# SavaRobotics/FoundationPose

Measured on AMD Instinct MI355X. Metric: pose-hypotheses/sec (render+refine+score), 252 hyp x 160x160, higher is better.
Workload: dtype f16

## Files before the change

foundationpose_amd/csrc/head_mlp.hip:

```cpp
#include "common.h"
#include "device_util.h"
#include <cstdlib>

#define HM_THREADS 512
#define HM_TILE 65536
#define HM_RED_OFF (2 * HM_TILE)
#define HM_LDS_BYTES (2 * HM_TILE + 4096)

struct HmCtx {
  int lane, wave, lr, lh;
  unsigned xo[8];
};

__device__ __forceinline__ void hm_gemm(const HmCtx &c, const f16 *w, const float *bias, const unsigned char *tile, floatx16 (&acc)[2][2]) {
  acc_from_bias(acc, bias, c.wave * 64, c.lh);
  const u32x4 *wp = reinterpret_cast<const u32x4 *>(w) + (size_t)(c.wave >> 1) * (32 * 4 * 64) + ((c.wave & 1) * 2) * 64 + c.lane;
  constexpr int D = 4;
  u32x4 wr[D][2];
#pragma unroll
  for (int d = 0; d < D; ++d)
#pragma unroll
    for (int i = 0; i < 2; ++i) wr[d][i] = wp[(d * 4 + i) * 64];
  const unsigned char *xb = tile + c.lr * 256;
  half8 bf[2][2];
#pragma unroll
  for (int j = 0; j < 2; ++j) bf[0][j] = *reinterpret_cast<const half8 *>(xb + j * 8192 + c.xo[0]);
#pragma unroll
  for (int k = 0; k < 32; ++k) {
    const int cur = k & 1, slot = k % D;
    half8 af[2];
#pragma unroll
    for (int i = 0; i < 2; ++i) af[i] = *reinterpret_cast<half8 *>(&wr[slot][i]);
    __builtin_amdgcn_sched_barrier(0);
    if (k + D < 32) {
#pragma unroll
      for (int i = 0; i < 2; ++i) wr[slot][i] = wp[((k + D) * 4 + i) * 64];
    }
    if (k + 1 < 32) {
      const int kn = k + 1;
#pragma unroll
      for (int j = 0; j < 2; ++j) bf[cur ^ 1][j] = *reinterpret_cast<const half8 *>(xb + (kn >> 3) * 16384 + j * 8192 + c.xo[kn & 7]);
    }
    __builtin_amdgcn_sched_barrier(0);
#pragma unroll
    for (int j = 0; j < 2; ++j)
#pragma unroll
      for (int i = 0; i < 2; ++i) acc[i][j] = __builtin_amdgcn_mfma_f32_32x32x16_f16(af[i], bf[cur][j], acc[i][j], 0, 0, 0);
  }
}

__device__ __forceinline__ unsigned hm_off(const HmCtx &c, int row, int i, int rg) {
  return (unsigned)((c.wave >> 1) * 16384 + row * 256 + ((((c.wave & 1) * 8 + i * 4 + rg) ^ (row & 15)) * 16) + c.lh * 8);
}

__device__ __forceinline__ void hm_residual_stats(const HmCtx &c, const unsigned char *res_tile, float *red, floatx16 (&acc)[2][2], float (&rstd)[2]) {
#pragma unroll
  for (int j = 0; j < 2; ++j) {
    const int row = j * 32 + c.lr;
#pragma unroll
    for (int i = 0; i < 2; ++i)
#pragma unroll
      for (int rg = 0; rg < 4; ++rg) {
        const half4 rq = *reinterpret_cast<const half4 *>(res_tile + hm_off(c, row, i, rg));
#pragma unroll
        for (int e = 0; e < 4; ++e) acc[i][j][rg * 4 + e] += (float)rq[e];
      }
  }
  float mean[2];
#pragma unroll
  for (int j = 0; j < 2; ++j) {
    float s = 0.f;
#pragma unroll
    for (int i = 0; i < 2; ++i)
#pragma unroll
      for (int e = 0; e < 16; ++e) s += acc[i][j][e];
    s += __shfl_xor(s, 32);
    if (c.lh == 0) red[c.wave * 64 + j * 32 + c.lr] = s;
  }
  __syncthreads();
#pragma unroll
  for (int j = 0; j < 2; ++j) {
    float s = 0.f;
#pragma unroll
    for (int w = 0; w < 8; ++w) s += red[w * 64 + j * 32 + c.lr];
    mean[j] = s * (1.f / 512.f);
  }
#pragma unroll
  for (int j = 0; j < 2; ++j) {
    float s = 0.f;
#pragma unroll
    for (int i = 0; i < 2; ++i)
#pragma unroll
      for (int e = 0; e < 16; ++e) {
        acc[i][j][e] -= mean[j];
        s += acc[i][j][e] * acc[i][j][e];
      }
    s += __shfl_xor(s, 32);
    if (c.lh == 0) red[512 + c.wave * 64 + j * 32 + c.lr] = s;
  }
  __syncthreads();
#pragma unroll
  for (int j = 0; j < 2; ++j) {
    float s = 0.f;
#pragma unroll
    for (int w = 0; w < 8; ++w) s += red[512 + w * 64 + j * 32 + c.lr];
    rstd[j] = rsqrtf(s * (1.f / 512.f) + 1e-5f);
  }
}

__global__ __launch_bounds__(HM_THREADS, 1) void head_mlp_kernel(HeadMlpArgs p) {
  extern __shared__ __attribute__((aligned(16))) unsigned char hm_smem[];
  HmCtx c;
  const int tid = threadIdx.x;
  c.lane = tid & 63;
  c.wave = __builtin_amdgcn_readfirstlane(tid >> 6);
  c.lr = c.lane & 31;
  c.lh = c.lane >> 5;
#pragma unroll
  for (int s = 0; s < 8; ++s) c.xo[s] = (unsigned)(((2 * s + c.lh) ^ (c.lr & 15)) * 16);
  const int m0 = blockIdx.x * 64;
  unsigned char *P = hm_smem, *Q = hm_smem + HM_TILE;
  float *red = reinterpret_cast<float *>(hm_smem + HM_RED_OFF);
  const unsigned lds0 = (unsigned)(size_t)(__attribute__((address_space(3))) void *)hm_smem;

  tok_tile_dma<64, 8>(p.att, m0, p.M, c.wave, c.lane, lds0);
  tok_tile_dma<64, 8>(p.tok, m0, p.M, c.wave, c.lane, lds0 + HM_TILE);
  wait_vm<8>();
  __syncthreads();

  floatx16 acc[2][2];
  float rstd[2];
  hm_gemm(c, p.w_out, p.b_out, P, acc);
  wait_vm<0>();
  __syncthreads();
  hm_residual_stats(c, Q, red, acc, rstd);
#pragma unroll
  for (int i = 0; i < 2; ++i)
#pragma unroll
    for (int rg = 0; rg < 4; ++rg) {
      const int col = c.wave * 64 + i * 32 + rg * 8 + c.lh * 4;
      const float4 gv = *reinterpret_cast<const float4 *>(p.g1 + col), bv = *reinterpret_cast<const float4 *>(p.be1 + col);
#pragma unroll
      for (int j = 0; j < 2; ++j) {
        half4 hv;
        hv[0] = (f16)(acc[i][j][rg * 4 + 0] * rstd[j] * gv.x + bv.x);
        hv[1] = (f16)(acc[i][j][rg * 4 + 1] * rstd[j] * gv.y + bv.y);
        hv[2] = (f16)(acc[i][j][rg * 4 + 2] * rstd[j] * gv.z + bv.z);
        hv[3] = (f16)(acc[i][j][rg * 4 + 3] * rstd[j] * gv.w + bv.w);
        *reinterpret_cast<half4 *>(Q + hm_off(c, j * 32 + c.lr, i, rg)) = hv;
      }
    }
  __syncthreads();
  hm_gemm(c, p.w1, p.b1, Q, acc);
#pragma unroll
  for (int i = 0; i < 2; ++i)
#pragma unroll
    for (int rg = 0; rg < 4; ++rg)
#pragma unroll
      for (int j = 0; j < 2; ++j) {
        half4 hv;
#pragma unroll
        for (int e = 0; e < 4; ++e) hv[e] = (f16)acc[i][j][rg * 4 + e];
        hv = __builtin_elementwise_max(hv, half4{(f16)0.f, (f16)0.f, (f16)0.f, (f16)0.f});
        *reinterpret_cast<half4 *>(P + hm_off(c, j * 32 + c.lr, i, rg)) = hv;
      }
  __syncthreads();
  hm_gemm(c, p.w2, p.b2, P, acc);
  hm_residual_stats(c, Q, red, acc, rstd);
#pragma unroll
  for (int j = 0; j < 2; ++j)
#pragma unroll
    for (int i = 0; i < 2; ++i)
#pragma unroll
      for (int rg = 0; rg < 4; ++rg) {
        float v[4];
#pragma unroll
        for (int e = 0; e < 4; ++e) v[e] = row16_sum(acc[i][j][rg * 4 + e] * rstd[j]);
        const int g = (m0 + j * 32 + (c.lr & 16)) >> 4;
        if ((c.lr & 15) == 0 && g * 16 < p.M)
          *reinterpret_cast<float4 *>(p.gsum + (size_t)g * 512 + c.wave * 64 + i * 32 + rg * 8 + c.lh * 4) = make_float4(v[0], v[1], v[2], v[3]);
      }
}


#define H2_ROWS 128
#ifdef HM_STAMP
__device__ unsigned long long g_hm_stamps[1024 * 8 * 8];
extern "C" __attribute__((visibility("default"))) int fp_dbg_hm_stamps(unsigned long long *host) {
  return hipMemcpyFromSymbol(host, HIP_SYMBOL(g_hm_stamps), sizeof(g_hm_stamps)) == hipSuccess ? 0 : -1;
}
#define HSTAMP(i) do { if (blockIdx.x < 1024 && c.lane == 0) g_hm_stamps[((size_t)blockIdx.x * 8 + c.wave) * 8 + (i)] = __builtin_amdgcn_s_memtime(); } while (0)
#else
#define HSTAMP(i) do { } while (0)
#endif
#define H2_SEG (H2_ROWS * 256)
#define H2_TILE (4 * H2_SEG)
#define H2_SLOT (H2_ROWS * 128)
#define H2_RING_OFF H2_TILE
#define H2_RED_OFF H2_RING_OFF
#define H2_LDS_BYTES (H2_TILE + 2 * H2_SLOT)

__device__ __forceinline__ void h2_ring_dma(const f16 *src, int m0, int M, int s8, int wave, int lane, unsigned slot_addr) {
#pragma unroll
  for (int u = 0; u < 2; ++u) {
    const int r8 = wave * 2 + u, row = r8 * 8 + (lane >> 3);
    const int m = min(m0 + row, M - 1);
    const unsigned voff = (unsigned)(((size_t)m * 512 + s8 * 64 + (((lane & 7) ^ (row & 7)) * 8)) * 2);
    glds16(src, voff, slot_addr + r8 * 1024);
  }
}

struct H2Ctx {
  int lane, wave, lr, lh;
};

template <bool RING, bool BIAS, typename Pre>
__device__ __forceinline__ void h2_gemm(const H2Ctx &c, const f16 *w, const float *bias, const unsigned char *smem, floatx16 (&acc)[2][4], Pre before_loop,
                                        unsigned lds0 = 0, const f16 *ring_src = nullptr, int m0 = 0, int M = 0) {
  const u32x4 *wp = reinterpret_cast<const u32x4 *>(w) + (size_t)(c.wave >> 1) * (32 * 4 * 64) + ((c.wave & 1) * 2) * 64 + c.lane;
  constexpr int D = 3;
  u32x4 wr[D][2];
#pragma unroll
  for (int d = 0; d < D; ++d)
#pragma unroll
    for (int i = 0; i < 2; ++i) wr[d][i] = wp[(d * 4 + i) * 64];
  __builtin_amdgcn_sched_barrier(0);
  if constexpr (RING) {
    wait_vm<6>();
    __syncthreads();
    h2_ring_dma(ring_src, m0, M, 1, c.wave, c.lane, lds0 + H2_RING_OFF + H2_SLOT);
  }
  floatx16 bvec[2];
  if constexpr (BIAS) {
#pragma unroll
    for (int i = 0; i < 2; ++i)
#pragma unroll
      for (int rg = 0; rg < 4; ++rg) {
        const float4 bv = *reinterpret_cast<const float4 *>(bias + c.wave * 64 + i * 32 + rg * 8 + c.lh * 4);
        bvec[i][rg * 4 + 0] = bv.x, bvec[i][rg * 4 + 1] = bv.y, bvec[i][rg * 4 + 2] = bv.z, bvec[i][rg * 4 + 3] = bv.w;
      }
  }
  __builtin_amdgcn_sched_barrier(0);
  before_loop();
  const unsigned char *xb = RING ? smem + H2_RING_OFF + c.lr * 128 + ((c.lh ^ (c.lr & 1)) * 16) : smem + c.lr * 256 + ((c.lh ^ (c.lr & 1)) * 16);
  const unsigned xe = (unsigned)(c.lr & (RING ? 6 : 14));
  auto frag_addr = [&](int k, int j) __attribute__((always_inline)) -> const unsigned char * {
    if constexpr (RING) return xb + ((k >> 2) & 1) * H2_SLOT + j * 4096 + (((unsigned)(2 * (k & 3)) ^ xe) << 4);
    else return xb + (k >> 3) * H2_SEG + j * 8192 + (((unsigned)(2 * (k & 7)) ^ xe) << 4);
  };
  half8 bf[4];
#pragma unroll
  for (int j = 0; j < 4; ++j) bf[j] = *reinterpret_cast<const half8 *>(frag_addr(0, j));
#pragma unroll
  for (int k = 0; k < 32; ++k) {
    const int slot = k % D;
    half8 af[2];
#pragma unroll
    for (int i = 0; i < 2; ++i) af[i] = *reinterpret_cast<half8 *>(&wr[slot][i]);
    __builtin_amdgcn_sched_barrier(0);
    if (k + D < 32) {
#pragma unroll
      for (int i = 0; i < 2; ++i) wr[slot][i] = wp[((k + D) * 4 + i) * 64];
    }
    __builtin_amdgcn_sched_barrier(0);
    const int kn = k + 1;
    const bool seg_edge = RING && (kn & 3) == 0 && kn < 32;
#pragma unroll
    for (int j = 0; j < 4; ++j) {
#pragma unroll
      for (int i = 0; i < 2; ++i) acc[i][j] = __builtin_amdgcn_mfma_f32_32x32x16_f16(af[i], bf[j], (BIAS && k == 0) ? bvec[i] : acc[i][j], 0, 0, 0);
      __builtin_amdgcn_sched_barrier(0);
      if (kn < 32 && !seg_edge) bf[j] = *reinterpret_cast<const half8 *>(frag_addr(kn, j));
      __builtin_amdgcn_sched_barrier(0);
    }
    if (seg_edge) {
      wait_vm_lgkm<8>();
      __syncthreads();
      if ((kn >> 2) + 1 < 8) h2_ring_dma(ring_src, m0, M, (kn >> 2) + 1, c.wave, c.lane, lds0 + H2_RING_OFF + (((kn >> 2) + 1) & 1) * H2_SLOT);
#pragma unroll
      for (int j = 0; j < 4; ++j) bf[j] = *reinterpret_cast<const half8 *>(frag_addr(kn, j));
    }
  }
}

__device__ __forceinline__ unsigned h2_off(const H2Ctx &c, int row, int i, int rg) {
  return (unsigned)((c.wave >> 1) * H2_SEG + row * 256 + ((((c.wave & 1) * 8 + i * 4 + rg) ^ (row & 15)) * 16) + c.lh * 8);
}
__device__ __forceinline__ H2Ctx h2_fresh(const H2Ctx &c0) {
  H2Ctx c = c0;
  asm volatile("" : "+v"(c.lr), "+v"(c.lh), "+v"(c.lane));
  return c;
}

__device__ __forceinline__ void h2_stats(const H2Ctx &c0, float *red, const floatx16 (&acc)[2][4], float (&mean)[4], float (&rstd)[4]) {
  H2Ctx c = c0;
  asm volatile("" : "+v"(c.lr));
#pragma unroll
  for (int j = 0; j < 4; ++j) {
    float s = 0.f, q = 0.f;
#pragma unroll
    for (int i = 0; i < 2; ++i)
#pragma unroll
      for (int e = 0; e < 16; ++e) {
        s += acc[i][j][e];
        q += acc[i][j][e] * acc[i][j][e];
      }
    s += __shfl_xor(s, 32);
    q += __shfl_xor(q, 32);
    if (c.lh == 0) *reinterpret_cast<float2 *>(&red[(c.wave * 128 + j * 32 + c.lr) * 2]) = make_float2(s, q);
  }
  __syncthreads();
#pragma unroll
  for (int j = 0; j < 4; ++j) {
    float s = 0.f, q = 0.f;
#pragma unroll
    for (int w = 0; w < 8; ++w) {
      const float2 v = *reinterpret_cast<const float2 *>(&red[(w * 128 + j * 32 + c.lr) * 2]);
      s += v.x;
      q += v.y;
    }
    mean[j] = s * (1.f / 512.f);
    rstd[j] = rsqrtf(fmaxf(q * (1.f / 512.f) - mean[j] * mean[j], 0.f) + 1e-5f);
  }
}

__global__ __launch_bounds__(HM_THREADS, 1) void head_mlp128_kernel(HeadMlpArgs p) {
  extern __shared__ __attribute__((aligned(16))) unsigned char h2_smem[];
  H2Ctx c;
  const int tid = threadIdx.x;
  c.lane = tid & 63;
  c.wave = __builtin_amdgcn_readfirstlane(tid >> 6);
  c.lr = c.lane & 31;
  c.lh = c.lane >> 5;
  const int m0 = blockIdx.x * H2_ROWS;
  unsigned char *Q = h2_smem;
  float *red = reinterpret_cast<float *>(h2_smem + H2_RED_OFF);
  const unsigned lds0 = (unsigned)(size_t)(__attribute__((address_space(3))) void *)h2_smem;

  HSTAMP(0);
  tok_tile_dma<H2_ROWS, 8, true>(p.tok, m0, p.M, c.wave, c.lane, lds0);
  h2_ring_dma(p.att, m0, p.M, 0, c.wave, c.lane, lds0 + H2_RING_OFF);
  floatx16 acc[2][4];
  float mean[4], rstd[4];
  h2_gemm<true, true>(c, p.w_out, p.b_out, h2_smem, acc, []() {}, lds0, p.att, m0, p.M);
  HSTAMP(1);
  __syncthreads();
  {
    const H2Ctx cr = h2_fresh(c);
#pragma unroll
    for (int j = 0; j < 4; ++j) {
      const int row = j * 32 + cr.lr;
#pragma unroll
      for (int i = 0; i < 2; ++i)
#pragma unroll
        for (int rg = 0; rg < 4; ++rg) {
          const half4 rq = *reinterpret_cast<const half4 *>(Q + h2_off(cr, row, i, rg));
#pragma unroll
          for (int e = 0; e < 4; ++e) acc[i][j][rg * 4 + e] += (float)rq[e];
        }
    }
  }
  h2_stats(c, red, acc, mean, rstd);
  const H2Ctx c1 = h2_fresh(c);
  float4 gv[2][4], bv[2][4];
#pragma unroll
  for (int i = 0; i < 2; ++i)
#pragma unroll
    for (int rg = 0; rg < 4; ++rg) {
      const int col = c.wave * 64 + i * 32 + rg * 8 + c1.lh * 4;
      gv[i][rg] = *reinterpret_cast<const float4 *>(p.g1 + col);
      bv[i][rg] = *reinterpret_cast<const float4 *>(p.be1 + col);
    }
#pragma unroll
  for (int j = 0; j < 4; ++j) {
    const float nm = -mean[j] * rstd[j];
#pragma unroll
    for (int i = 0; i < 2; ++i)
#pragma unroll
      for (int rg = 0; rg < 4; ++rg) {
        half4 hv;
        hv[0] = (f16)__builtin_fmaf(__builtin_fmaf(acc[i][j][rg * 4 + 0], rstd[j], nm), gv[i][rg].x, bv[i][rg].x);
        hv[1] = (f16)__builtin_fmaf(__builtin_fmaf(acc[i][j][rg * 4 + 1], rstd[j], nm), gv[i][rg].y, bv[i][rg].y);
        hv[2] = (f16)__builtin_fmaf(__builtin_fmaf(acc[i][j][rg * 4 + 2], rstd[j], nm), gv[i][rg].z, bv[i][rg].z);
        hv[3] = (f16)__builtin_fmaf(__builtin_fmaf(acc[i][j][rg * 4 + 3], rstd[j], nm), gv[i][rg].w, bv[i][rg].w);
        *reinterpret_cast<half4 *>(Q + h2_off(c1, j * 32 + c1.lr, i, rg)) = hv;
      }
  }
  HSTAMP(2);
  h2_gemm<false, true>(c, p.w1, p.b1, h2_smem, acc, [&]() __attribute__((always_inline)) { __syncthreads(); });
  HSTAMP(3);
  half4 ff[2][4][4];
#pragma unroll
  for (int i = 0; i < 2; ++i)
#pragma unroll
    for (int j = 0; j < 4; ++j)
#pragma unroll
      for (int rg = 0; rg < 4; ++rg) {
        half4 hv;
#pragma unroll
        for (int e = 0; e < 4; ++e) hv[e] = (f16)acc[i][j][rg * 4 + e];
        ff[i][j][rg] = __builtin_elementwise_max(hv, half4{(f16)0.f, (f16)0.f, (f16)0.f, (f16)0.f});
      }
  const H2Ctx c2 = h2_fresh(c);
  float4 b2v[2][4];
#pragma unroll
  for (int i = 0; i < 2; ++i)
#pragma unroll
    for (int rg = 0; rg < 4; ++rg) b2v[i][rg] = *reinterpret_cast<const float4 *>(p.b2 + c.wave * 64 + i * 32 + rg * 8 + c2.lh * 4);
  __syncthreads();
#pragma unroll
  for (int i = 0; i < 2; ++i)
#pragma unroll
    for (int rg = 0; rg < 4; ++rg)
#pragma unroll
      for (int j = 0; j < 4; ++j) {
        unsigned char *q = Q + h2_off(c2, j * 32 + c2.lr, i, rg);
        const half4 xq = *reinterpret_cast<const half4 *>(q);
        acc[i][j][rg * 4 + 0] = b2v[i][rg].x + (float)xq[0];
        acc[i][j][rg * 4 + 1] = b2v[i][rg].y + (float)xq[1];
        acc[i][j][rg * 4 + 2] = b2v[i][rg].z + (float)xq[2];
        acc[i][j][rg * 4 + 3] = b2v[i][rg].w + (float)xq[3];
        *reinterpret_cast<half4 *>(q) = ff[i][j][rg];
      }
  HSTAMP(4);
  h2_gemm<false, false>(c, p.w2, nullptr, h2_smem, acc, [&]() __attribute__((always_inline)) { __syncthreads(); });
  HSTAMP(5);
  h2_stats(c, red, acc, mean, rstd);
  {
    const H2Ctx c3 = h2_fresh(c);
    unsigned char *tb = Q + c.wave * 16384;
#pragma unroll
    for (int h = 0; h < 2; ++h) {
#pragma unroll
      for (int jj = 0; jj < 2; ++jj) {
        const int j = 2 * h + jj, row = jj * 32 + c3.lr;
        const float nm = -mean[j] * rstd[j];
#pragma unroll
        for (int i = 0; i < 2; ++i)
#pragma unroll
          for (int rg = 0; rg < 4; ++rg)
            *reinterpret_cast<float4 *>(tb + row * 256 + (((i * 8 + rg * 2 + c3.lh) ^ (row & 15)) * 16)) =
                make_float4(__builtin_fmaf(acc[i][j][rg * 4 + 0], rstd[j], nm), __builtin_fmaf(acc[i][j][rg * 4 + 1], rstd[j], nm),
                            __builtin_fmaf(acc[i][j][rg * 4 + 2], rstd[j], nm), __builtin_fmaf(acc[i][j][rg * 4 + 3], rstd[j], nm));
      }
      __builtin_amdgcn_fence(__ATOMIC_RELEASE, "wavefront");
#pragma unroll
      for (int gq = 0; gq < 4; ++gq) {
        float sum = 0.f;
#pragma unroll
        for (int t = 0; t < 16; ++t) sum += *reinterpret_cast<const float *>(tb + (gq * 16 + t) * 256 + ((((c3.lane >> 2) ^ t)) * 16) + (c3.lane & 3) * 4);
        const int g = (m0 + h * 64 + gq * 16) >> 4;
        if (g * 16 < p.M) p.gsum[(size_t)g * 512 + c.wave * 64 + c3.lane] = sum;
      }
      __builtin_amdgcn_fence(__ATOMIC_RELEASE, "wavefront");
    }
  }
  HSTAMP(6);
}

void head_mlp_kernel_lds(std::vector<KernelLds> &v) {
  v.push_back({(const void *)head_mlp_kernel, HM_LDS_BYTES});
  v.push_back({(const void *)head_mlp128_kernel, H2_LDS_BYTES});
}

int launch_head_mlp(fp_ctx *ctx, const HeadMlpArgs &a, hipStream_t s) {
  FP_REQUIRE(a.att && a.tok && a.w_out && a.w1 && a.w2 && a.b_out && a.b1 && a.b2 && a.g1 && a.be1 && a.gsum, "head_mlp: null argument");
  FP_REQUIRE(a.M >= 0 && a.M % 16 == 0, "head_mlp: M=%d must be a multiple of 16", a.M);
  if (a.M == 0) return FP_OK;
  FP_REQUIRE((double)a.M * 1024.0 < 4294967296.0, "head_mlp: M=%d too large for 32-bit lane offsets", a.M);
  ProfScope ps(ctx, s, "linear", 3.0 * 2.0 * (double)a.M * 512.0 * 512.0);
  static const bool form64 = fp_env_set("FP_HEADMLP64");
  if (form64 || a.M <= 1600) hipLaunchKernelGGL(head_mlp_kernel, dim3((a.M + 63) / 64), dim3(HM_THREADS), HM_LDS_BYTES, s, a);
  else hipLaunchKernelGGL(head_mlp128_kernel, dim3((a.M + H2_ROWS - 1) / H2_ROWS), dim3(HM_THREADS), H2_LDS_BYTES, s, a);
  FP_CHECK_HIP(hipGetLastError());
  return FP_OK;
}
```

Measured before the change: 7366.

## Template head MLP kernel on row count; stream token tile alongside attention ring

The 128-row head MLP body becomes a template over rows per block, and a 64-row variant is added with launch bounds allowing four blocks per CU. It is only selected through an environment variable. On the default path the token tile is no longer loaded up front; it is fetched piecewise inside the first GEMM's ring loop at each segment edge, which hides that load behind MFMA work. The wait counts change to match, and LayerNorm parameter loads are restructured to lower register pressure. The risk is extra vmcnt bookkeeping and a dependence on correct wait placement before the residual read.

```diff
diff --git a/foundationpose_amd/csrc/head_mlp.hip b/foundationpose_amd/csrc/head_mlp.hip
--- a/foundationpose_amd/csrc/head_mlp.hip
+++ b/foundationpose_amd/csrc/head_mlp.hip
@@ -184,6 +184,7 @@
 
 
 #define H2_ROWS 128
+#define H3_ROWS 64
 #ifdef HM_STAMP
 __device__ unsigned long long g_hm_stamps[1024 * 8 * 8];
 extern "C" __attribute__((visibility("default"))) int fp_dbg_hm_stamps(unsigned long long *host) {
@@ -193,30 +194,47 @@
 #else
 #define HSTAMP(i) do { } while (0)
 #endif
-#define H2_SEG (H2_ROWS * 256)
-#define H2_TILE (4 * H2_SEG)
-#define H2_SLOT (H2_ROWS * 128)
-#define H2_RING_OFF H2_TILE
-#define H2_RED_OFF H2_RING_OFF
-#define H2_LDS_BYTES (H2_TILE + 2 * H2_SLOT)
-
+#define H2_SEG(R) ((R) * 256)
+#define H2_TILE(R) (4 * H2_SEG(R))
+#define H2_SLOT(R) ((R) * 128)
+#define H2_RING_OFF(R) H2_TILE(R)
+#define H2_RED_OFF(R) H2_RING_OFF(R)
+#define H2_LDS_BYTES(R) (H2_TILE(R) + 2 * H2_SLOT(R))
+
+template <int R>
 __device__ __forceinline__ void h2_ring_dma(const f16 *src, int m0, int M, int s8, int wave, int lane, unsigned slot_addr) {
-#pragma unroll
-  for (int u = 0; u < 2; ++u) {
-    const int r8 = wave * 2 + u, row = r8 * 8 + (lane >> 3);
+  constexpr int U = R / 64;
+#pragma unroll
+  for (int u = 0; u < U; ++u) {
+    const int r8 = wave * U + u, row = r8 * 8 + (lane >> 3);
     const int m = min(m0 + row, M - 1);
     const unsigned voff = (unsigned)(((size_t)m * 512 + s8 * 64 + (((lane & 7) ^ (row & 7)) * 8)) * 2);
     glds16(src, voff, slot_addr + r8 * 1024);
   }
 }
 
+template <int R>
+__device__ __forceinline__ void h2_tile_piece(const f16 *src, int m0, int M, int piece, int wave, int lane, unsigned lds0) {
+  constexpr int U = R / 32, T = R / 64;
+  asm volatile("" : "+v"(lane));
+#pragma unroll
+  for (int t = 0; t < T; ++t) {
+    const int idx = piece * T + t, seg = idx / U, u = idx % U;
+    const int r4 = wave * U + u, row = r4 * 4 + (lane >> 4);
+    const int m = min(m0 + row, M - 1);
+    const unsigned voff = (unsigned)(((size_t)m * 512 + seg * 128 + (((lane & 15) ^ (row & 15)) * 8)) * 2);
+    glds16(src, voff, lds0 + seg * H2_SEG(R) + r4 * 1024);
+  }
+}
+
 struct H2Ctx {
   int lane, wave, lr, lh;
 };
 
-template <bool RING, bool BIAS, typename Pre>
-__device__ __forceinline__ void h2_gemm(const H2Ctx &c, const f16 *w, const float *bias, const unsigned char *smem, floatx16 (&acc)[2][4], Pre before_loop,
-                                        unsigned lds0 = 0, const f16 *ring_src = nullptr, int m0 = 0, int M = 0) {
+template <int R, bool RING, bool BIAS, typename Pre>
+__device__ __forceinline__ void h2_gemm(const H2Ctx &c, const f16 *w, const float *bias, const unsigned char *smem, floatx16 (&acc)[2][R / 32], Pre before_loop,
+                                        unsigned lds0 = 0, const f16 *ring_src = nullptr, const f16 *tile_src = nullptr, int m0 = 0, int M = 0) {
+  constexpr int NJ = R / 32, PIECE = R / 64;
   const u32x4 *wp = reinterpret_cast<const u32x4 *>(w) + (size_t)(c.wave >> 1) * (32 * 4 * 64) + ((c.wave & 1) * 2) * 64 + c.lane;
   constexpr int D = 3;
   u32x4 wr[D][2];
@@ -228,7 +246,8 @@
   if constexpr (RING) {
     wait_vm<6>();
     __syncthreads();
-    h2_ring_dma(ring_src, m0, M, 1, c.wave, c.lane, lds0 + H2_RING_OFF + H2_SLOT);
+    h2_ring_dma<R>(ring_src, m0, M, 1, c.wave, c.lane, lds0 + H2_RING_OFF(R) + H2_SLOT(R));
+    h2_tile_piece<R>(tile_src, m0, M, 0, c.wave, c.lane, lds0);
   }
   floatx16 bvec[2];
   if constexpr (BIAS) {
@@ -242,15 +261,15 @@
   }
   __builtin_amdgcn_sched_barrier(0);
   before_loop();
-  const unsigned char *xb = RING ? smem + H2_RING_OFF + c.lr * 128 + ((c.lh ^ (c.lr & 1)) * 16) : smem + c.lr * 256 + ((c.lh ^ (c.lr & 1)) * 16);
+  const unsigned char *xb = RING ? smem + H2_RING_OFF(R) + c.lr * 128 + ((c.lh ^ (c.lr & 1)) * 16) : smem + c.lr * 256 + ((c.lh ^ (c.lr & 1)) * 16);
   const unsigned xe = (unsigned)(c.lr & (RING ? 6 : 14));
   auto frag_addr = [&](int k, int j) __attribute__((always_inline)) -> const unsigned char * {
-    if constexpr (RING) return xb + ((k >> 2) & 1) * H2_SLOT + j * 4096 + (((unsigned)(2 * (k & 3)) ^ xe) << 4);
-    else return xb + (k >> 3) * H2_SEG + j * 8192 + (((unsigned)(2 * (k & 7)) ^ xe) << 4);
+    if constexpr (RING) return xb + ((k >> 2) & 1) * H2_SLOT(R) + j * 4096 + (((unsigned)(2 * (k & 3)) ^ xe) << 4);
+    else return xb + (k >> 3) * H2_SEG(R) + j * 8192 + (((unsigned)(2 * (k & 7)) ^ xe) << 4);
   };
-  half8 bf[4];
-#pragma unroll
-  for (int j = 0; j < 4; ++j) bf[j] = *reinterpret_cast<const half8 *>(frag_addr(0, j));
+  half8 bf[NJ];
+#pragma unroll
+  for (int j = 0; j < NJ; ++j) bf[j] = *reinterpret_cast<const half8 *>(frag_addr(0, j));
 #pragma unroll
   for (int k = 0; k < 32; ++k) {
     const int slot = k % D;
@@ -266,7 +285,7 @@
     const int kn = k + 1;
     const bool seg_edge = RING && (kn & 3) == 0 && kn < 32;
 #pragma unroll
-    for (int j = 0; j < 4; ++j) {
+    for (int j = 0; j < NJ; ++j) {
 #pragma unroll
       for (int i = 0; i < 2; ++i) acc[i][j] = __builtin_amdgcn_mfma_f32_32x32x16_f16(af[i], bf[j], (BIAS && k == 0) ? bvec[i] : acc[i][j], 0, 0, 0);
       __builtin_amdgcn_sched_barrier(0);
@@ -274,17 +293,19 @@
       __builtin_amdgcn_sched_barrier(0);
     }
     if (seg_edge) {
-      wait_vm_lgkm<8>();
+      wait_vm_lgkm<8 + PIECE>();
       __syncthreads();
-      if ((kn >> 2) + 1 < 8) h2_ring_dma(ring_src, m0, M, (kn >> 2) + 1, c.wave, c.lane, lds0 + H2_RING_OFF + (((kn >> 2) + 1) & 1) * H2_SLOT);
-#pragma unroll
-      for (int j = 0; j < 4; ++j) bf[j] = *reinterpret_cast<const half8 *>(frag_addr(kn, j));
-    }
-  }
-}
-
+      if ((kn >> 2) + 1 < 8) h2_ring_dma<R>(ring_src, m0, M, (kn >> 2) + 1, c.wave, c.lane, lds0 + H2_RING_OFF(R) + (((kn >> 2) + 1) & 1) * H2_SLOT(R));
+      h2_tile_piece<R>(tile_src, m0, M, kn >> 2, c.wave, c.lane, lds0);
+#pragma unroll
+      for (int j = 0; j < NJ; ++j) bf[j] = *reinterpret_cast<const half8 *>(frag_addr(kn, j));
+    }
+  }
+}
+
+template <int R>
 __device__ __forceinline__ unsigned h2_off(const H2Ctx &c, int row, int i, int rg) {
-  return (unsigned)((c.wave >> 1) * H2_SEG + row * 256 + ((((c.wave & 1) * 8 + i * 4 + rg) ^ (row & 15)) * 16) + c.lh * 8);
+  return (unsigned)((c.wave >> 1) * H2_SEG(R) + row * 256 + ((((c.wave & 1) * 8 + i * 4 + rg) ^ (row & 15)) * 16) + c.lh * 8);
 }
 __device__ __forceinline__ H2Ctx h2_fresh(const H2Ctx &c0) {
   H2Ctx c = c0;
@@ -292,11 +313,12 @@
   return c;
 }
 
-__device__ __forceinline__ void h2_stats(const H2Ctx &c0, float *red, const floatx16 (&acc)[2][4], float (&mean)[4], float (&rstd)[4]) {
+template <int NJ>
+__device__ __forceinline__ void h2_stats(const H2Ctx &c0, float *red, const floatx16 (&acc)[2][NJ], float (&mean)[NJ], float (&rstd)[NJ]) {
   H2Ctx c = c0;
   asm volatile("" : "+v"(c.lr));
 #pragma unroll
-  for (int j = 0; j < 4; ++j) {
+  for (int j = 0; j < NJ; ++j) {
     float s = 0.f, q = 0.f;
 #pragma unroll
     for (int i = 0; i < 2; ++i)
@@ -307,15 +329,15 @@
       }
     s += __shfl_xor(s, 32);
     q += __shfl_xor(q, 32);
-    if (c.lh == 0) *reinterpret_cast<float2 *>(&red[(c.wave * 128 + j * 32 + c.lr) * 2]) = make_float2(s, q);
-  }
-  __syncthreads();
-#pragma unroll
-  for (int j = 0; j < 4; ++j) {
+    if (c.lh == 0) *reinterpret_cast<float2 *>(&red[(c.wave * (NJ * 32) + j * 32 + c.lr) * 2]) = make_float2(s, q);
+  }
+  __syncthreads();
+#pragma unroll
+  for (int j = 0; j < NJ; ++j) {
     float s = 0.f, q = 0.f;
 #pragma unroll
     for (int w = 0; w < 8; ++w) {
-      const float2 v = *reinterpret_cast<const float2 *>(&red[(w * 128 + j * 32 + c.lr) * 2]);
+      const float2 v = *reinterpret_cast<const float2 *>(&red[(w * (NJ * 32) + j * 32 + c.lr) * 2]);
       s += v.x;
       q += v.y;
     }
@@ -324,37 +346,39 @@
   }
 }
 
-__global__ __launch_bounds__(HM_THREADS, 1) void head_mlp128_kernel(HeadMlpArgs p) {
+template <int R>
+__device__ __forceinline__ void h2_body(const HeadMlpArgs &p) {
   extern __shared__ __attribute__((aligned(16))) unsigned char h2_smem[];
+  constexpr int NJ = R / 32;
   H2Ctx c;
   const int tid = threadIdx.x;
   c.lane = tid & 63;
   c.wave = __builtin_amdgcn_readfirstlane(tid >> 6);
   c.lr = c.lane & 31;
   c.lh = c.lane >> 5;
-  const int m0 = blockIdx.x * H2_ROWS;
+  const int m0 = blockIdx.x * R;
   unsigned char *Q = h2_smem;
-  float *red = reinterpret_cast<float *>(h2_smem + H2_RED_OFF);
+  float *red = reinterpret_cast<float *>(h2_smem + H2_RED_OFF(R));
   const unsigned lds0 = (unsigned)(size_t)(__attribute__((address_space(3))) void *)h2_smem;
 
   HSTAMP(0);
-  tok_tile_dma<H2_ROWS, 8, true>(p.tok, m0, p.M, c.wave, c.lane, lds0);
-  h2_ring_dma(p.att, m0, p.M, 0, c.wave, c.lane, lds0 + H2_RING_OFF);
-  floatx16 acc[2][4];
-  float mean[4], rstd[4];
-  h2_gemm<true, true>(c, p.w_out, p.b_out, h2_smem, acc, []() {}, lds0, p.att, m0, p.M);
+  h2_ring_dma<R>(p.att, m0, p.M, 0, c.wave, c.lane, lds0 + H2_RING_OFF(R));
+  floatx16 acc[2][NJ];
+  float mean[NJ], rstd[NJ];
+  h2_gemm<R, true, true>(c, p.w_out, p.b_out, h2_smem, acc, []() {}, lds0, p.att, p.tok, m0, p.M);
   HSTAMP(1);
+  wait_vm<0>();
   __syncthreads();
   {
     const H2Ctx cr = h2_fresh(c);
 #pragma unroll
-    for (int j = 0; j < 4; ++j) {
+    for (int j = 0; j < NJ; ++j) {
       const int row = j * 32 + cr.lr;
 #pragma unroll
       for (int i = 0; i < 2; ++i)
 #pragma unroll
         for (int rg = 0; rg < 4; ++rg) {
-          const half4 rq = *reinterpret_cast<const half4 *>(Q + h2_off(cr, row, i, rg));
+          const half4 rq = *reinterpret_cast<const half4 *>(Q + h2_off<R>(cr, row, i, rg));
 #pragma unroll
           for (int e = 0; e < 4; ++e) acc[i][j][rg * 4 + e] += (float)rq[e];
         }
@@ -362,78 +386,81 @@
   }
   h2_stats(c, red, acc, mean, rstd);
   const H2Ctx c1 = h2_fresh(c);
-  float4 gv[2][4], bv[2][4];
+  float nm[NJ];
+#pragma unroll
+  for (int j = 0; j < NJ; ++j) nm[j] = -mean[j] * rstd[j];
 #pragma unroll
   for (int i = 0; i < 2; ++i)
 #pragma unroll
     for (int rg = 0; rg < 4; ++rg) {
       const int col = c.wave * 64 + i * 32 + rg * 8 + c1.lh * 4;
-      gv[i][rg] = *reinterpret_cast<const float4 *>(p.g1 + col);
-      bv[i][rg] = *reinterpret_cast<const float4 *>(p.be1 + col);
-    }
-#pragma unroll
-  for (int j = 0; j < 4; ++j) {
-    const float nm = -mean[j] * rstd[j];
-#pragma unroll
-    for (int i = 0; i < 2; ++i)
+      const float4 gv = *reinterpret_cast<const float4 *>(p.g1 + col), bv = *reinterpret_cast<const float4 *>(p.be1 + col);
+#pragma unroll
+      for (int j = 0; j < NJ; ++j) {
+        half4 hv;
+        hv[0] = (f16)__builtin_fmaf(__builtin_fmaf(acc[i][j][rg * 4 + 0], rstd[j], nm[j]), gv.x, bv.x);
+        hv[1] = (f16)__builtin_fmaf(__builtin_fmaf(acc[i][j][rg * 4 + 1], rstd[j], nm[j]), gv.y, bv.y);
+        hv[2] = (f16)__builtin_fmaf(__builtin_fmaf(acc[i][j][rg * 4 + 2], rstd[j], nm[j]), gv.z, bv.z);
+        hv[3] = (f16)__builtin_fmaf(__builtin_fmaf(acc[i][j][rg * 4 + 3], rstd[j], nm[j]), gv.w, bv.w);
+        *reinterpret_cast<half4 *>(Q + h2_off<R>(c1, j * 32 + c1.lr, i, rg)) = hv;
+      }
+    }
+  HSTAMP(2);
+  h2_gemm<R, false, true>(c, p.w1, p.b1, h2_smem, acc, [&]() __attribute__((always_inline)) { __syncthreads(); });
+  HSTAMP(3);
+  half4 ff[2][NJ][4];
+#pragma unroll
+  for (int i = 0; i < 2; ++i)
+#pragma unroll
+    for (int j = 0; j < NJ; ++j)
 #pragma unroll
       for (int rg = 0; rg < 4; ++rg) {
         half4 hv;
-        hv[0] = (f16)__builtin_fmaf(__builtin_fmaf(acc[i][j][rg * 4 + 0], rstd[j], nm), gv[i][rg].x, bv[i][rg].x);
-        hv[1] = (f16)__builtin_fmaf(__builtin_fmaf(acc[i][j][rg * 4 + 1], rstd[j], nm), gv[i][rg].y, bv[i][rg].y);
-        hv[2] = (f16)__builtin_fmaf(__builtin_fmaf(acc[i][j][rg * 4 + 2], rstd[j], nm), gv[i][rg].z, bv[i][rg].z);
-        hv[3] = (f16)__builtin_fmaf(__builtin_fmaf(acc[i][j][rg * 4 + 3], rstd[j], nm), gv[i][rg].w, bv[i][rg].w);
-        *reinterpret_cast<half4 *>(Q + h2_off(c1, j * 32 + c1.lr, i, rg)) = hv;
-      }
-  }
-  HSTAMP(2);
-  h2_gemm<false, true>(c, p.w1, p.b1, h2_smem, acc, [&]() __attribute__((always_inline)) { __syncthreads(); });
-  HSTAMP(3);
-  half4 ff[2][4][4];
-#pragma unroll
-  for (int i = 0; i < 2; ++i)
-#pragma unroll
-    for (int j = 0; j < 4; ++j)
-#pragma unroll
-      for (int rg = 0; rg < 4; ++rg) {
-        half4 hv;
 #pragma unroll
         for (int e = 0; e < 4; ++e) hv[e] = (f16)acc[i][j][rg * 4 + e];
         ff[i][j][rg] = __builtin_elementwise_max(hv, half4{(f16)0.f, (f16)0.f, (f16)0.f, (f16)0.f});
       }
   const H2Ctx c2 = h2_fresh(c);
-  float4 b2v[2][4];
+  constexpr bool B2_EARLY = NJ == 4;
+  float4 b2e[2][4];
+  if constexpr (B2_EARLY) {
+#pragma unroll
+    for (int i = 0; i < 2; ++i)
+#pragma unroll
+      for (int rg = 0; rg < 4; ++rg) b2e[i][rg] = *reinterpret_cast<const float4 *>(p.b2 + c.wave * 64 + i * 32 + rg * 8 + c2.lh * 4);
+  }
+  __syncthreads();
 #pragma unroll
   for (int i = 0; i < 2; ++i)
 #pragma unroll
-    for (int rg = 0; rg < 4; ++rg) b2v[i][rg] = *reinterpret_cast<const float4 *>(p.b2 + c.wave * 64 + i * 32 + rg * 8 + c2.lh * 4);
-  __syncthreads();
-#pragma unroll
-  for (int i = 0; i < 2; ++i)
-#pragma unroll
-    for (int rg = 0; rg < 4; ++rg)
-#pragma unroll
-      for (int j = 0; j < 4; ++j) {
-        unsigned char *q = Q + h2_off(c2, j * 32 + c2.lr, i, rg);
+    for (int rg = 0; rg < 4; ++rg) {
+      float4 b2v;
+      if constexpr (B2_EARLY) b2v = b2e[i][rg];
+      else b2v = *reinterpret_cast<const float4 *>(p.b2 + c.wave * 64 + i * 32 + rg * 8 + c2.lh * 4);
+#pragma unroll
+      for (int j = 0; j < NJ; ++j) {
+        unsigned char *q = Q + h2_off<R>(c2, j * 32 + c2.lr, i, rg);
         const half4 xq = *reinterpret_cast<const half4 *>(q);
-        acc[i][j][rg * 4 + 0] = b2v[i][rg].x + (float)xq[0];
-        acc[i][j][rg * 4 + 1] = b2v[i][rg].y + (float)xq[1];
-        acc[i][j][rg * 4 + 2] = b2v[i][rg].z + (float)xq[2];
-        acc[i][j][rg * 4 + 3] = b2v[i][rg].w + (float)xq[3];
+        acc[i][j][rg * 4 + 0] = b2v.x + (float)xq[0];
+        acc[i][j][rg * 4 + 1] = b2v.y + (float)xq[1];
+        acc[i][j][rg * 4 + 2] = b2v.z + (float)xq[2];
+        acc[i][j][rg * 4 + 3] = b2v.w + (float)xq[3];
         *reinterpret_cast<half4 *>(q) = ff[i][j][rg];
       }
+    }
   HSTAMP(4);
-  h2_gemm<false, false>(c, p.w2, nullptr, h2_smem, acc, [&]() __attribute__((always_inline)) { __syncthreads(); });
+  h2_gemm<R, false, false>(c, p.w2, nullptr, h2_smem, acc, [&]() __attribute__((always_inline)) { __syncthreads(); });
   HSTAMP(5);
   h2_stats(c, red, acc, mean, rstd);
   {
+    constexpr int JH = NJ / 2;
     const H2Ctx c3 = h2_fresh(c);
-    unsigned char *tb = Q + c.wave * 16384;
+    unsigned char *tb = Q + c.wave * (H2_TILE(R) / 8);
 #pragma unroll
     for (int h = 0; h < 2; ++h) {
 #pragma unroll
-      for (int jj = 0; jj < 2; ++jj) {
-        const int j = 2 * h + jj, row = jj * 32 + c3.lr;
+      for (int jj = 0; jj < JH; ++jj) {
+        const int j = JH * h + jj, row = jj * 32 + c3.lr;
         const float nm = -mean[j] * rstd[j];
 #pragma unroll
         for (int i = 0; i < 2; ++i)
@@ -445,11 +472,11 @@
       }
       __builtin_amdgcn_fence(__ATOMIC_RELEASE, "wavefront");
 #pragma unroll
-      for (int gq = 0; gq < 4; ++gq) {
+      for (int gq = 0; gq < 2 * JH; ++gq) {
         float sum = 0.f;
 #pragma unroll
         for (int t = 0; t < 16; ++t) sum += *reinterpret_cast<const float *>(tb + (gq * 16 + t) * 256 + ((((c3.lane >> 2) ^ t)) * 16) + (c3.lane & 3) * 4);
-        const int g = (m0 + h * 64 + gq * 16) >> 4;
+        const int g = (m0 + h * (R / 2) + gq * 16) >> 4;
         if (g * 16 < p.M) p.gsum[(size_t)g * 512 + c.wave * 64 + c3.lane] = sum;
       }
       __builtin_amdgcn_fence(__ATOMIC_RELEASE, "wavefront");
@@ -457,10 +484,14 @@
   }
   HSTAMP(6);
 }
+
+__global__ __launch_bounds__(HM_THREADS, 1) void head_mlp128_kernel(HeadMlpArgs p) { h2_body<H2_ROWS>(p); }
+__global__ __launch_bounds__(HM_THREADS, 4) void head_mlp64x2_kernel(HeadMlpArgs p) { h2_body<H3_ROWS>(p); }
 
 void head_mlp_kernel_lds(std::vector<KernelLds> &v) {
   v.push_back({(const void *)head_mlp_kernel, HM_LDS_BYTES});
-  v.push_back({(const void *)head_mlp128_kernel, H2_LDS_BYTES});
+  v.push_back({(const void *)head_mlp128_kernel, H2_LDS_BYTES(H2_ROWS)});
+  v.push_back({(const void *)head_mlp64x2_kernel, H2_LDS_BYTES(H3_ROWS)});
 }
 
 int launch_head_mlp(fp_ctx *ctx, const HeadMlpArgs &a, hipStream_t s) {
@@ -470,8 +501,10 @@
   FP_REQUIRE((double)a.M * 1024.0 < 4294967296.0, "head_mlp: M=%d too large for 32-bit lane offsets", a.M);
   ProfScope ps(ctx, s, "linear", 3.0 * 2.0 * (double)a.M * 512.0 * 512.0);
   static const bool form64 = fp_env_set("FP_HEADMLP64");
+  static const bool form64x2 = fp_env_set("FP_HEADMLP64X2");
   if (form64 || a.M <= 1600) hipLaunchKernelGGL(head_mlp_kernel, dim3((a.M + 63) / 64), dim3(HM_THREADS), HM_LDS_BYTES, s, a);
-  else hipLaunchKernelGGL(head_mlp128_kernel, dim3((a.M + H2_ROWS - 1) / H2_ROWS), dim3(HM_THREADS), H2_LDS_BYTES, s, a);
+  else if (form64x2) hipLaunchKernelGGL(head_mlp64x2_kernel, dim3((a.M + H3_ROWS - 1) / H3_ROWS), dim3(HM_THREADS), H2_LDS_BYTES(H3_ROWS), s, a);
+  else hipLaunchKernelGGL(head_mlp128_kernel, dim3((a.M + H2_ROWS - 1) / H2_ROWS), dim3(HM_THREADS), H2_LDS_BYTES(H2_ROWS), s, a);
   FP_CHECK_HIP(hipGetLastError());
   return FP_OK;
 }
```

Result: no change. 7357, median of 2 (-0.1%).
